# NYXFLOWER/TIP

Measured on AMD Instinct MI355X. Metric: D-D edges aggregated/sec (encoder fwd+bwd), higher is better.
Workload: dtype f32; 1 GPU; TIP-cat full encoder, BioSNAP (645 drugs, 19081 proteins, R=1097), 1xMI355X config; mod=cat, directed_dd_edges=8326508, relations=1097, parallelism=single GPU, launch=hipGraph replay of the captured step, rccl_ranks=0

## Files before the change

### tip_amd/csrc/tipk_gemm.hip

```cpp
#include <stdlib.h>
#include "tipk_common.h"
#include "tipk_slabs.h"

namespace {

typedef float f32x16 __attribute__((ext_vector_type(16)));

constexpr int BK = 32;
constexpr int PAD = 4;

struct GemmArgs {
    int64_t m, n, k, kbatch, ksplit, kchunk;
    const float* a; int64_t a_sm, a_sk, a_sq, a_sz;
    const float* b; int64_t b_sk, b_sn, b_sq, b_sz;
    float* c; int64_t c_sm, c_sz, c_ss;
    const float* c_in; int64_t cin_sm, cin_sz;
    float alpha;
    int relu;
};

typedef unsigned int u32;

__device__ __forceinline__ float ldg(const float* base, u32 byte_off) {
    return *reinterpret_cast<const float*>(reinterpret_cast<const char*>(base) + byte_off);
}
__device__ __forceinline__ float4 ldg4(const float* base, u32 byte_off) {
    return *reinterpret_cast<const float4*>(reinterpret_cast<const char*>(base) + byte_off);
}

template <int ROWS>
struct TileLoader {
    static constexpr int PER = ROWS * BK / 256;
    float v[PER];
    __device__ __forceinline__ static void coord(bool kfast, int i, int t, int& r, int& kk) {
        r = kfast ? t / BK + (256 / BK) * i : t % ROWS;
        kk = kfast ? t % BK : t / ROWS + (256 / ROWS) * i;
    }
    __device__ __forceinline__ void load(bool kfast, const float* tile, u32 s_r, u32 s_k, int rows_left, int k_left, int t) {
#pragma unroll
        for (int i = 0; i < PER; ++i) {
            int r, kk;
            coord(kfast, i, t, r, kk);
            v[i] = (r < rows_left && kk < k_left) ? ldg(tile, ((u32)r * s_r + (u32)kk * s_k) * 4u) : 0.f;
        }
    }
    __device__ __forceinline__ void store(bool kfast, float (*lds)[ROWS + PAD], int t) const {
#pragma unroll
        for (int i = 0; i < PER; ++i) {
            int r, kk;
            coord(kfast, i, t, r, kk);
            lds[kk][r] = v[i];
        }
    }
};

template <int WM, int WN, int NBUF, int R = 1>
__device__ __forceinline__ void gemm_body(const GemmArgs& g, int64_t bx, int64_t by, int64_t bz, float* smem,
                                          const bool A_KFAST, const bool B_KFAST) {
    constexpr int BM = WM * 32 * R, BN = WN * 32 * R;
    static_assert(WM * WN == 4, "4 waves per workgroup");
    float (*As)[BK][BM + PAD] = reinterpret_cast<float (*)[BK][BM + PAD]>(smem);
    float (*Bs)[BK][BN + PAD] = reinterpret_cast<float (*)[BK][BN + PAD]>(smem + NBUF * BK * (BM + PAD));

    const int t = threadIdx.x;
    const int lane = t & 63, wid = t >> 6;
    const int wm = wid / WN, wn = wid % WN;
    const int64_t m0 = by * BM, n0 = bx * BN;
    const int64_t z = bz / g.ksplit, slab = bz % g.ksplit;
    const int64_t k_lo = slab * g.kchunk;
    const int64_t k_hi = (k_lo + g.kchunk < g.k) ? k_lo + g.kchunk : g.k;
    const int tiles_per_q = (k_hi > k_lo) ? (int)((k_hi - k_lo + BK - 1) / BK) : 0;
    const int n_tiles = tiles_per_q * (int)g.kbatch;

    const float* a_z = g.a + z * g.a_sz + m0 * g.a_sm + k_lo * g.a_sk;
    const float* b_z = g.b + z * g.b_sz + n0 * g.b_sn + k_lo * g.b_sk;
    const u32 a_sm = (u32)g.a_sm, a_sk = (u32)g.a_sk, b_sn = (u32)g.b_sn, b_sk = (u32)g.b_sk;
    const int m_left = (int)(g.m - m0 < BM ? g.m - m0 : BM), n_left = (int)(g.n - n0 < BN ? g.n - n0 : BN);

    TileLoader<BM> la;
    TileLoader<BN> lb;
    f32x16 acc[R][R];
#pragma unroll
    for (int a = 0; a < R; ++a)
#pragma unroll
        for (int b = 0; b < R; ++b)
#pragma unroll
            for (int i = 0; i < 16; ++i) acc[a][b][i] = 0.f;

    auto fetch = [&](int tile) {
        const int q = tile / tiles_per_q;
        const int kt = tile - q * tiles_per_q;
        const int k_left = (int)(k_hi - k_lo) - kt * BK;
        la.load(A_KFAST, a_z + (int64_t)q * g.a_sq + (int64_t)kt * BK * g.a_sk, a_sm, a_sk, m_left, k_left, t);
        lb.load(B_KFAST, b_z + (int64_t)q * g.b_sq + (int64_t)kt * BK * g.b_sk, b_sn, b_sk, n_left, k_left, t);
    };

    if (n_tiles > 0) fetch(0);
    for (int tile = 0; tile < n_tiles; ++tile) {
        const int buf = NBUF == 2 ? (tile & 1) : 0;
        if (NBUF == 1 && tile > 0) __syncthreads();
        la.store(A_KFAST, As[buf], t);
        lb.store(B_KFAST, Bs[buf], t);
        __syncthreads();
        if (tile + 1 < n_tiles) fetch(tile + 1);
        const int row = lane & 31, kh = lane >> 5;
#pragma unroll
        for (int kk = 0; kk < BK / 2; ++kk) {
            float av[R], bv[R];
#pragma unroll
            for (int a = 0; a < R; ++a) av[a] = As[buf][2 * kk + kh][(wm * R + a) * 32 + row];
#pragma unroll
            for (int b = 0; b < R; ++b) bv[b] = Bs[buf][2 * kk + kh][(wn * R + b) * 32 + row];
#pragma unroll
            for (int a = 0; a < R; ++a)
#pragma unroll
                for (int b = 0; b < R; ++b)
                    acc[a][b] = __builtin_amdgcn_mfma_f32_32x32x2f32(av[a], bv[b], acc[a][b], 0, 0, 0);
        }
    }

    float* c_z = g.c + z * g.c_sz + slab * g.c_ss;
    const float* cin_z = g.c_in ? g.c_in + z * g.cin_sz : nullptr;
#pragma unroll
    for (int a = 0; a < R; ++a) {
#pragma unroll
        for (int b = 0; b < R; ++b) {
            const int64_t col = n0 + (wn * R + b) * 32 + (lane & 31);
            if (col >= g.n) continue;
#pragma unroll
            for (int r = 0; r < 16; ++r) {
                const int64_t rowi = m0 + (wm * R + a) * 32 + (r & 3) + 8 * (r >> 2) + 4 * (lane >> 5);
                if (rowi < g.m) {
                    float v = g.alpha * acc[a][b][r];
                    if (cin_z) v += cin_z[rowi * g.cin_sm + col];
                    if (g.relu) v = fmaxf(v, 0.f);
                    c_z[rowi * g.c_sm + col] = v;
                }
            }
        }
    }
}

template <int WM, int WN, bool A_KFAST, bool B_KFAST, int NBUF, int R = 1>
__global__ __launch_bounds__(256) void gemm_f32_kernel(GemmArgs g) {
    __shared__ __attribute__((aligned(16))) float smem[NBUF * BK * (WM * 32 * R + WN * 32 * R + 2 * PAD)];
    gemm_body<WM, WN, NBUF, R>(g, blockIdx.x, blockIdx.y, blockIdx.z, smem, A_KFAST, B_KFAST);
}

constexpr int THIN_K_NT = 4;

__device__ __forceinline__ f32x16 zero16() {
    f32x16 z;
#pragma unroll
    for (int i = 0; i < 16; ++i) z[i] = 0.f;
    return z;
}

__device__ __forceinline__ void store_tile(const GemmArgs& g, const f32x16& acc, float* c_z, const float* cin_z,
                                           int64_t m0, int64_t n0, int lane) {
    const int64_t col = n0 + (lane & 31);
    if (col >= g.n) return;
#pragma unroll
    for (int r = 0; r < 16; ++r) {
        const int64_t rowi = m0 + (r & 3) + 8 * (r >> 2) + 4 * (lane >> 5);
        if (rowi < g.m) {
            float v = g.alpha * acc[r];
            if (cin_z) v += cin_z[rowi * g.cin_sm + col];
            if (g.relu) v = fmaxf(v, 0.f);
            c_z[rowi * g.c_sm + col] = v;
        }
    }
}

__device__ __forceinline__ float and_mask(float v, u32 mask) { return __uint_as_float(__float_as_uint(v) & mask); }
__device__ __forceinline__ int uniform(int v) { return __builtin_amdgcn_readfirstlane(v); }

__device__ __forceinline__ void store_tile32(const GemmArgs& g, const f32x16& acc, float* c_z, const float* cin_z,
                                             int m0, int n0, int lane) {
    const int col = n0 + (lane & 31);
    if (col >= (int)g.n) return;
    float* c_t = c_z + (int64_t)m0 * g.c_sm + n0;
    const float* cin_t = cin_z ? cin_z + (int64_t)m0 * g.cin_sm + n0 : nullptr;
    const u32 c_sm = (u32)g.c_sm * 4u, cin_sm = (u32)g.cin_sm * 4u;
    const u32 cb = (u32)(lane & 31) * 4u;
#pragma unroll
    for (int r = 0; r < 16; ++r) {
        const int rl = (r & 3) + 8 * (r >> 2) + 4 * (lane >> 5);
        if (m0 + rl < (int)g.m) {
            float v = g.alpha * acc[r];
            if (cin_t) v += ldg(cin_t, (u32)rl * cin_sm + cb);
            if (g.relu) v = fmaxf(v, 0.f);
            *reinterpret_cast<float*>(reinterpret_cast<char*>(c_t) + ((u32)rl * c_sm + cb)) = v;
        }
    }
}

template <bool WIDE>
__device__ __forceinline__ void gemm_thin_k_body(const GemmArgs& g, int64_t block) {
    const int lane = threadIdx.x & 63;
    const int row = lane & 31, kh = lane >> 5;
    const int M = (int)g.m, N = (int)g.n, K = (int)g.k;
    const int m_tiles = (M + 31) / 32;
    const int n_chunks = (N + 32 * THIN_K_NT - 1) / (32 * THIN_K_NT);
    const int gw = uniform((int)block * 4 + (int)(threadIdx.x >> 6));
    const int z = uniform(gw / (m_tiles * n_chunks));
    const int rem = gw - z * (m_tiles * n_chunks);
    const int chunk = uniform(rem / m_tiles), mt = uniform(rem - chunk * m_tiles);
    if (z >= g.kbatch) return;
    const int m0 = mt * 32;
    const float* __restrict__ a_z = g.a + z * g.a_sz;
    const float* __restrict__ b_z = g.b + z * g.b_sz;
    float* c_z = g.c + z * g.c_sz;
    const float* cin_z = g.c_in ? g.c_in + z * g.cin_sz : nullptr;
    const u32 a_sk = (u32)g.a_sk * 4u, b_sk = (u32)g.b_sk * 4u;
    const u32 aoff = (u32)(m0 + row < M ? m0 + row : M - 1) * (u32)g.a_sm * 4u;
    float av[16];
    u32 koff[16];
    const bool a_vec = WIDE && g.a_sk == 1 && (g.a_sm & 3) == 0 && (g.a_sz & 3) == 0 && K == 32 &&
                       (reinterpret_cast<uintptr_t>(g.a) & 15) == 0;
    if (a_vec) {
#pragma unroll
        for (int q = 0; q < 4; ++q) {
            const float4 t = ldg4(a_z, aoff + (u32)(16 * kh + 4 * q) * 4u);
            av[4 * q + 0] = t.x; av[4 * q + 1] = t.y; av[4 * q + 2] = t.z; av[4 * q + 3] = t.w;
        }
    }
#pragma unroll
    for (int kk = 0; kk < 16; ++kk) {
        const int k = WIDE ? 16 * kh + kk : 2 * kk + kh;
        const u32 kc = (u32)(k < K ? k : K - 1);
        if (!a_vec) av[kk] = and_mask(ldg(a_z, aoff + kc * a_sk), k < K ? 0xffffffffu : 0u);
        koff[kk] = kc * b_sk;
    }
    const int nb = chunk * (32 * THIN_K_NT);
    if (WIDE) {
        const int col = nb + 4 * row;
        const u32 cc = (u32)(col < N ? col : N - 4) * 4u;
        float4 b4[16];
#pragma unroll
        for (int kk = 0; kk < 16; ++kk) b4[kk] = ldg4(b_z, koff[kk] + cc);
        __builtin_amdgcn_sched_barrier(0);
        f32x16 a0 = zero16(), a1 = zero16(), a2 = zero16(), a3 = zero16();
#pragma unroll
        for (int kk = 0; kk < 16; ++kk) {
            a0 = __builtin_amdgcn_mfma_f32_32x32x2f32(av[kk], b4[kk].x, a0, 0, 0, 0);
            a1 = __builtin_amdgcn_mfma_f32_32x32x2f32(av[kk], b4[kk].y, a1, 0, 0, 0);
            a2 = __builtin_amdgcn_mfma_f32_32x32x2f32(av[kk], b4[kk].z, a2, 0, 0, 0);
            a3 = __builtin_amdgcn_mfma_f32_32x32x2f32(av[kk], b4[kk].w, a3, 0, 0, 0);
        }
        if (col >= N) return;
        float* c_t = c_z + (int64_t)m0 * g.c_sm + nb;
        const float* cin_t = cin_z ? cin_z + (int64_t)m0 * g.cin_sm + nb : nullptr;
        const u32 c_sm = (u32)g.c_sm * 4u, cin_sm = (u32)g.cin_sm * 4u, cb = (u32)row * 16u;
#pragma unroll
        for (int r = 0; r < 16; ++r) {
            const int rl = (r & 3) + 8 * (r >> 2) + 4 * kh;
            if (m0 + rl < M) {
                float4 v = make_float4(g.alpha * a0[r], g.alpha * a1[r], g.alpha * a2[r], g.alpha * a3[r]);
                if (cin_t) {
                    const float4 ci = ldg4(cin_t, (u32)rl * cin_sm + cb);
                    v.x += ci.x; v.y += ci.y; v.z += ci.z; v.w += ci.w;
                }
                if (g.relu) { v.x = fmaxf(v.x, 0.f); v.y = fmaxf(v.y, 0.f); v.z = fmaxf(v.z, 0.f); v.w = fmaxf(v.w, 0.f); }
                *reinterpret_cast<float4*>(reinterpret_cast<char*>(c_t) + ((u32)rl * c_sm + cb)) = v;
            }
        }
        return;
    }
    float bt[THIN_K_NT][16];
#pragma unroll
    for (int j = 0; j < THIN_K_NT; ++j) {
        const int col = nb + 32 * j + row;
        const u32 cc = (u32)(col < N ? col : N - 1) * 4u;
#pragma unroll
        for (int kk = 0; kk < 16; ++kk) bt[j][kk] = ldg(b_z, koff[kk] + cc);
    }
    __builtin_amdgcn_sched_barrier(0);
#pragma unroll
    for (int j = 0; j < THIN_K_NT; ++j) {
        f32x16 acc = zero16();
#pragma unroll
        for (int kk = 0; kk < 16; ++kk) acc = __builtin_amdgcn_mfma_f32_32x32x2f32(av[kk], bt[j][kk], acc, 0, 0, 0);
        store_tile32(g, acc, c_z, cin_z, m0, nb + 32 * j, lane);
    }
}

__device__ __forceinline__ void gemm_thin_m_body(const GemmArgs& g, int64_t block) {
    const int lane = threadIdx.x & 63;
    const int row = lane & 31, kh = lane >> 5;
    const int M = (int)g.m, N = (int)g.n;
    const int n_tiles = (N + 31) / 32;
    const int gw = uniform((int)block * 4 + (int)(threadIdx.x >> 6));
    const int zs = uniform(gw / n_tiles);
    const int nt = gw - zs * n_tiles;
    const int z = uniform(zs / (int)g.ksplit);
    const int slab = zs - z * (int)g.ksplit;
    if (z >= g.kbatch) return;
    const int k_lo = slab * (int)g.kchunk;
    const int k_hi = (k_lo + (int)g.kchunk < (int)g.k) ? k_lo + (int)g.kchunk : (int)g.k;
    const float* __restrict__ a_z = g.a + z * g.a_sz;
    const float* __restrict__ b_z = g.b + z * g.b_sz;
    const int n0 = nt * 32;
    const int col = n0 + row;
    const u32 cc = (u32)(col < N ? col : N - 1) * 4u;
    const u32 a_sk = (u32)g.a_sk * 4u, b_sk = (u32)g.b_sk * 4u;
    const u32 ar = (u32)(row < M ? row : M - 1) * (u32)g.a_sm * 4u;
    float a0[16], b0[16], a1[16], b1[16];
#define TIPK_LOAD_AB(A, B, K0)                                                 \
    _Pragma("unroll") for (int kk = 0; kk < 16; ++kk) {                        \
        const int k_ = (K0) + 2 * kk + kh;                                     \
        const u32 kc_ = (u32)(k_ < k_hi ? k_ : k_hi - 1);                      \
        A[kk] = ldg(a_z, ar + kc_ * a_sk);                                     \
        B[kk] = ldg(b_z, kc_ * b_sk + cc);                                     \
    }                                                                          \
    __builtin_amdgcn_sched_barrier(0);
#define TIPK_MMA(A, B, K0)                                                     \
    _Pragma("unroll") for (int kk = 0; kk < 16; ++kk)                          \
        acc = __builtin_amdgcn_mfma_f32_32x32x2f32(and_mask(A[kk], (K0) + 2 * kk + kh < k_hi ? 0xffffffffu : 0u), \
                                                   B[kk], acc, 0, 0, 0);       \
    __builtin_amdgcn_sched_barrier(0);
    f32x16 acc = zero16();
    if (k_lo < k_hi) {
        TIPK_LOAD_AB(a0, b0, k_lo)
#pragma unroll 1
        for (int k0 = k_lo; k0 < k_hi; k0 += 64) {
            TIPK_LOAD_AB(a1, b1, k0 + 32)
            TIPK_MMA(a0, b0, k0)
            TIPK_LOAD_AB(a0, b0, k0 + 64)
            TIPK_MMA(a1, b1, k0 + 32)
        }
    }
#undef TIPK_LOAD_AB
#undef TIPK_MMA
    float* c_z = g.c + z * g.c_sz + (int64_t)slab * g.c_ss;
    const float* cin_z = g.c_in ? g.c_in + z * g.cin_sz : nullptr;
    store_tile32(g, acc, c_z, cin_z, 0, n0, lane);
}

__device__ __forceinline__ void gemm_kk_body(const GemmArgs& g, int64_t block) {
    const int lane = threadIdx.x & 63;
    const int row = lane & 31, kh = lane >> 5;
    const int M = (int)g.m, N = (int)g.n;
    const int m_tiles = (M + 31) / 32;
    const int gw = uniform((int)block * 4 + (int)(threadIdx.x >> 6));
    const int zs = uniform(gw / m_tiles);
    const int mt = gw - zs * m_tiles;
    const int z = uniform(zs / (int)g.ksplit);
    const int slab = zs - z * (int)g.ksplit;
    if (z >= g.kbatch) return;
    const int k_lo = slab * (int)g.kchunk;
    const int k_hi = (k_lo + (int)g.kchunk < (int)g.k) ? k_lo + (int)g.kchunk : (int)g.k;
    const int m0 = mt * 32;
    const float* __restrict__ a_z = g.a + z * g.a_sz;
    const float* __restrict__ b_z = g.b + z * g.b_sz;
    const u32 ar = (u32)(m0 + row < M ? m0 + row : M - 1) * (u32)g.a_sm * 4u;
    const u32 br = (u32)(row < N ? row : N - 1) * (u32)g.b_sn * 4u;
    float4 a0[4], b0[4], a1[4], b1[4];
#define TIPK_LOAD_AB(A, B, K0)                                                 \
    _Pragma("unroll") for (int q = 0; q < 4; ++q) {                            \
        const int k_ = (K0) + 8 * q + 4 * kh;                                  \
        const u32 kc_ = (u32)(k_ < k_hi ? k_ : k_hi - 4) * 4u;                 \
        A[q] = ldg4(a_z, ar + kc_);                                            \
        B[q] = ldg4(b_z, br + kc_);                                            \
    }                                                                          \
    __builtin_amdgcn_sched_barrier(0);
#define TIPK_KK_STEP(A, B, K0)                                                 \
    _Pragma("unroll") for (int q = 0; q < 4; ++q) {                            \
        const u32 mk_ = (K0) + 8 * q + 4 * kh < k_hi ? 0xffffffffu : 0u;       \
        acc = __builtin_amdgcn_mfma_f32_32x32x2f32(and_mask(A[q].x, mk_), B[q].x, acc, 0, 0, 0); \
        acc = __builtin_amdgcn_mfma_f32_32x32x2f32(and_mask(A[q].y, mk_), B[q].y, acc, 0, 0, 0); \
        acc = __builtin_amdgcn_mfma_f32_32x32x2f32(and_mask(A[q].z, mk_), B[q].z, acc, 0, 0, 0); \
        acc = __builtin_amdgcn_mfma_f32_32x32x2f32(and_mask(A[q].w, mk_), B[q].w, acc, 0, 0, 0); \
    }                                                                          \
    __builtin_amdgcn_sched_barrier(0);
    f32x16 acc = zero16();
    if (k_lo < k_hi) {
        TIPK_LOAD_AB(a0, b0, k_lo)
#pragma unroll 1
        for (int k0 = k_lo; k0 < k_hi; k0 += 64) {
            TIPK_LOAD_AB(a1, b1, k0 + 32)
            TIPK_KK_STEP(a0, b0, k0)
            TIPK_LOAD_AB(a0, b0, k0 + 64)
            TIPK_KK_STEP(a1, b1, k0 + 32)
        }
    }
#undef TIPK_LOAD_AB
#undef TIPK_KK_STEP
    float* c_z = g.c + z * g.c_sz + (int64_t)slab * g.c_ss;
    const float* cin_z = g.c_in ? g.c_in + z * g.cin_sz : nullptr;
    store_tile32(g, acc, c_z, cin_z, m0, 0, lane);
}

enum { STREAM_NONE = 0, STREAM_THIN_K = 1, STREAM_THIN_M = 2, STREAM_KK = 3, STREAM_THIN_K4 = 4 };

inline bool thin_k_wide_ok(const GemmArgs& g, int64_t batch) {
    static_assert(THIN_K_NT == 4, "the wide body owns four interleaved tiles");
    if ((g.n & 3) || ((g.b_sk | g.c_sm | g.b_sz | g.c_sz) & 3)) return false;
    if (g.c_in && ((g.cin_sm | g.cin_sz) & 3)) return false;
    return ((reinterpret_cast<uintptr_t>(g.b) | reinterpret_cast<uintptr_t>(g.c) | reinterpret_cast<uintptr_t>(g.c_in)) & 15) == 0;
}

inline int stream_kind(const GemmArgs& g, int64_t batch) {
    if (g.kbatch != 1) return STREAM_NONE;
    const bool big = g.m * g.n >= (1 << 20) || g.n * g.k >= (1 << 20) || g.m * g.k >= (1 << 20);
    if (!big) return STREAM_NONE;
    const int64_t lim = 0x3fffffffLL;
    if (g.a_sm < 0 || g.a_sk < 0 || g.b_sk < 0 || g.b_sn < 0 || g.m > lim || g.n > lim || g.k > lim) return STREAM_NONE;
    if ((g.m - 1) * g.a_sm + (g.k - 1) * g.a_sk >= lim || (g.k - 1) * g.b_sk + (g.n - 1) * g.b_sn >= lim) return STREAM_NONE;
    if (g.c_sm < 0 || g.cin_sm < 0 || 32 * g.c_sm >= lim || 32 * g.cin_sm >= lim) return STREAM_NONE;
    if (g.k <= 32 && g.ksplit == 1 && g.b_sn == 1 && (g.m >= 256 || (g.m >= 8 && g.n >= (1 << 16))) && g.n >= 1024)
        return (thin_k_wide_ok(g, batch) && !tipk_option(TIPK_OPT_GEMM_THIN_K_NARROW)) ? STREAM_THIN_K4 : STREAM_THIN_K;
    if (g.m <= 32 && g.b_sn == 1 && g.n >= 1024 && g.k >= 256) return STREAM_THIN_M;
    if (tipk_option(TIPK_OPT_GEMM_STREAM_KK) && g.n <= 32 && g.a_sk == 1 && g.b_sk == 1 && g.m >= 256 && g.k >= 1024 && g.k % 4 == 0 && g.a_sm % 4 == 0 &&
        g.b_sn % 4 == 0 && g.a_sz % 4 == 0 && g.b_sz % 4 == 0 && (reinterpret_cast<uintptr_t>(g.a) & 15) == 0 &&
        (reinterpret_cast<uintptr_t>(g.b) & 15) == 0)
        return STREAM_KK;
    return STREAM_NONE;
}

inline int64_t stream_blocks(int kind, const GemmArgs& g, int64_t batch) {
    int64_t waves = 0;
    if (kind == STREAM_THIN_K || kind == STREAM_THIN_K4) waves = batch * tipk_ceil_div(g.m, 32) * tipk_ceil_div(g.n, 32 * THIN_K_NT);
    if (kind == STREAM_THIN_M) waves = batch * g.ksplit * tipk_ceil_div(g.n, 32);
    if (kind == STREAM_KK) waves = batch * g.ksplit * tipk_ceil_div(g.m, 32);
    return tipk_ceil_div(waves, 4);
}

template <int KIND>
__global__ __launch_bounds__(256) void gemm_stream_kernel(GemmArgs g) {
    if (KIND == STREAM_THIN_K) gemm_thin_k_body<false>(g, blockIdx.x);
    if (KIND == STREAM_THIN_K4) gemm_thin_k_body<true>(g, blockIdx.x);
    if (KIND == STREAM_THIN_M) gemm_thin_m_body(g, blockIdx.x);
    if (KIND == STREAM_KK) gemm_kk_body(g, blockIdx.x);
}

constexpr int GROUP_MAX = TIPK_GROUP_MAX;

struct GemmGroupArgs {
    int count;
    int first_block[GROUP_MAX + 1];
    int cfg[GROUP_MAX];
    int gx[GROUP_MAX], gy[GROUP_MAX];
    GemmArgs g[GROUP_MAX];
};

__global__ __launch_bounds__(256) void gemm_f32_group_kernel(GemmGroupArgs ga) {
    __shared__ __attribute__((aligned(16))) float smem[2 * BK * (160 + 2 * PAD)];
    GemmArgs g = ga.g[0];
    int first = 0, gx = ga.gx[0], gy = ga.gy[0], cfg = ga.cfg[0];
#pragma unroll
    for (int q = 1; q < GROUP_MAX; ++q)
        if (q < ga.count && (int)blockIdx.x >= ga.first_block[q]) {
            g = ga.g[q]; first = ga.first_block[q]; gx = ga.gx[q]; gy = ga.gy[q]; cfg = ga.cfg[q];
        }
    const int local = (int)blockIdx.x - first;
    const int64_t bx = local % gx, by = (local / gx) % gy, bz = local / (gx * gy);
    const bool akf = (cfg & 2) != 0, bkf = (cfg & 1) != 0;
    switch (cfg >= 100 ? cfg : cfg >> 2) {
    case 0: gemm_body<4, 1, 2>(g, bx, by, bz, smem, akf, bkf); break;
    case 1: gemm_body<1, 4, 2>(g, bx, by, bz, smem, akf, bkf); break;
    case 2: gemm_body<2, 2, 2>(g, bx, by, bz, smem, akf, bkf); break;
    case 100 + STREAM_THIN_M: gemm_thin_m_body(g, local); break;
    case 100 + STREAM_KK: gemm_kk_body(g, local); break;
    }
}

template <int WM, int WN, int R = 1>
int launch(const GemmArgs& g, int64_t batch, hipStream_t st) {
    constexpr int BM = WM * 32 * R, BN = WN * 32 * R;
    const int64_t gx = tipk_ceil_div(g.n, BN), gy = tipk_ceil_div(g.m, BM), gz = batch * g.ksplit;
    if (gx > 0x7fffffffLL || gy > 65535 || gz > 65535) return TIPK_EUNSUPPORTED;
    dim3 grid((unsigned)gx, (unsigned)gy, (unsigned)gz), block(256);
    const bool akf = g.a_sk == 1 || g.a_sm != 1;
    const bool bkf = g.b_sk == 1 && g.b_sn != 1;
    const bool one_tile = g.kbatch == 1 && g.kchunk <= BK;
#define TIPK_GEMM_GO(A, B)                                                                              \
    do {                                                                                                \
        if (one_tile) hipLaunchKernelGGL((gemm_f32_kernel<WM, WN, A, B, 1, R>), grid, block, 0, st, g); \
        else hipLaunchKernelGGL((gemm_f32_kernel<WM, WN, A, B, (R > 1 ? 1 : 2), R>), grid, block, 0, st, g); \
    } while (0)
    if (akf && bkf) TIPK_GEMM_GO(true, true);
    else if (akf) TIPK_GEMM_GO(true, false);
    else if (bkf) TIPK_GEMM_GO(false, true);
    else TIPK_GEMM_GO(false, false);
#undef TIPK_GEMM_GO
    TIPK_RETURN_LAUNCH();
}

template <int LANES>
__global__ __launch_bounds__(64 * LANES) void sum_slabs_kernel(const float* __restrict__ in, int64_t n_slabs,
                                                               int64_t slab_stride, int64_t count, float alpha,
                                                               int accumulate, const float* __restrict__ row_scale,
                                                               int64_t cols, const float* __restrict__ addend,
                                                               int relu, float* __restrict__ out) {
    __shared__ float red[LANES][64];
    const int e = threadIdx.x & 63, j = threadIdx.x >> 6;
    const int64_t i = (int64_t)blockIdx.x * 64 + e;
    float s = 0.f;
    if (i < count) {
        const float* p = in + i;
        int64_t k = j;
        for (; k + 3 * LANES < n_slabs; k += 4 * LANES) {
            const float v0 = p[k * slab_stride], v1 = p[(k + LANES) * slab_stride];
            const float v2 = p[(k + 2 * LANES) * slab_stride], v3 = p[(k + 3 * LANES) * slab_stride];
            s += v0; s += v1; s += v2; s += v3;
        }
        for (; k < n_slabs; k += LANES) s += p[k * slab_stride];
    }
    red[j][e] = s;
    __syncthreads();
    if (j == 0 && i < count) {
        s = red[0][e];
#pragma unroll
        for (int q = 1; q < LANES; ++q) s += red[q][e];
        s *= alpha;
        if (row_scale) s *= row_scale[i / cols];
        if (addend) s += addend[i];
        if (accumulate) s += out[i];
        if (relu) s = fmaxf(s, 0.f);
        out[i] = s;
    }
}

struct SlabGroupArgs {
    int count;
    int first_block[GROUP_MAX + 1];
    SlabArgs s[GROUP_MAX];
};

__global__ __launch_bounds__(1024) void sum_slabs_group_kernel(SlabGroupArgs sa) {
    __shared__ float red[1024];
    SlabArgs a = sa.s[0];
    int first = 0;
#pragma unroll
    for (int q = 1; q < GROUP_MAX; ++q)
        if (q < sa.count && (int)blockIdx.x >= sa.first_block[q]) { a = sa.s[q]; first = sa.first_block[q]; }
    slab_sum_body(a, (int)blockIdx.x - first, red);
}

constexpr int WGK_MAX = 4, WGK_SUMS = 3, WGK_WAVES = 16;

struct WgkJob {
    const float* a; int64_t a_sm, a_sk, a_sq, a_sz;
    const float* b; int64_t b_sk, b_sn, b_sq, b_sz;
    const float* a2; int64_t a2_sm, a2_sk;
    const float* b2; int64_t b2_sk, b2_sn;
    float* c; int64_t c_sm, c_sz;
    const float* c_in; int64_t cin_sm, cin_sz;
    const float* gate; int64_t gate_sm, gate_sz;
    int m, n, k, k2, kbatch;
    int mt, nt;
    int tiles_q, n_kt, per, nw;
    int vec1, vec2;
    float alpha; int relu;
};
struct WgkArgs {
    int n_gemm, n_sum;
    int first[WGK_MAX + WGK_SUMS + 1];
    WgkJob g[WGK_MAX];
    SlabArgs s[WGK_SUMS];
};

__global__ __launch_bounds__(1024) void gemm_wgk_group_kernel(WgkArgs wa) {
    __shared__ __attribute__((aligned(16))) float red[WGK_WAVES * 1024];
    const int blk = (int)blockIdx.x;
    if (blk >= wa.first[WGK_MAX]) {
        SlabArgs sa = wa.s[0];
        int first = wa.first[WGK_MAX];
#pragma unroll
        for (int q = 1; q < WGK_SUMS; ++q)
            if (q < wa.n_sum && blk >= wa.first[WGK_MAX + q]) { sa = wa.s[q]; first = wa.first[WGK_MAX + q]; }
        slab_sum_body(sa, blk - first, red);
        return;
    }
    WgkJob g = wa.g[0];
    int first = 0;
#pragma unroll
    for (int q = 1; q < WGK_MAX; ++q)
        if (q < wa.n_gemm && blk >= wa.first[q]) { g = wa.g[q]; first = wa.first[q]; }
    const int local = blk - first;
    const int nt_i = local % g.nt, mt_i = (local / g.nt) % g.mt, z = local / (g.nt * g.mt);
    const int t = threadIdx.x, lane = t & 63, row = lane & 31, kh = lane >> 5;
    const int w = uniform(t >> 6);
    const int m0 = mt_i * 32, n0 = nt_i * 32;
    const int n_first = g.kbatch * g.tiles_q;
    const u32 am = (u32)(m0 + row < g.m ? m0 + row : g.m - 1), bn = (u32)(n0 + row < g.n ? n0 + row : g.n - 1);
    const u32 m_mask = m0 + row < g.m ? 0xffffffffu : 0u;

    f32x16 acc = zero16();
    float a0[16], b0[16], a1[16], b1[16];
    int left0 = 0, left1 = 0;
    auto load = [&](int tile, float (&av)[16], float (&bv)[16], int& left) {
        const bool second = tile >= n_first;
        const int tq = second ? tile - n_first : tile;
        const int q = second ? 0 : tq / g.tiles_q;
        const int kt = second ? tq : tq - q * g.tiles_q;
        const int kk_total = second ? g.k2 : g.k;
        const int k0 = kt * 32;
        left = kk_total - k0 < 32 ? kk_total - k0 : 32;
        const float* ap = second ? g.a2 : g.a + (int64_t)z * g.a_sz + (int64_t)q * g.a_sq;
        const float* bp = second ? g.b2 : g.b + (int64_t)z * g.b_sz + (int64_t)q * g.b_sq;
        const u32 s_am = (u32)(second ? g.a2_sm : g.a_sm), s_ak = (u32)(second ? g.a2_sk : g.a_sk);
        const u32 s_bk = (u32)(second ? g.b2_sk : g.b_sk), s_bn = (u32)(second ? g.b2_sn : g.b_sn);
        const u32 ao = am * s_am, bo = bn * s_bn;
        if (second ? g.vec2 : g.vec1) {
#pragma unroll
            for (int j = 0; j < 4; ++j) {
                const int kb = 16 * kh + 4 * j;
                const u32 kc = (u32)(k0 + (kb < left ? kb : left - 4));
                const float4 xa = ldg4(ap, (ao + kc) * 4u), xb = ldg4(bp, (bo + kc) * 4u);
                av[4 * j] = xa.x; av[4 * j + 1] = xa.y; av[4 * j + 2] = xa.z; av[4 * j + 3] = xa.w;
                bv[4 * j] = xb.x; bv[4 * j + 1] = xb.y; bv[4 * j + 2] = xb.z; bv[4 * j + 3] = xb.w;
            }
            left = -left;
            return;
        }
#pragma unroll
        for (int kk = 0; kk < 16; ++kk) {
            const int kl = 2 * kk + kh;
            const u32 kc = (u32)(k0 + (kl < left ? kl : left - 1));
            av[kk] = ldg(ap, (ao + kc * s_ak) * 4u);
            bv[kk] = ldg(bp, (kc * s_bk + bo) * 4u);
        }
    };
    auto mma = [&](const float (&av)[16], const float (&bv)[16], int left) {
        const int lim = left < 0 ? -left - 16 * kh : left - kh;
        const int step = left < 0 ? 1 : 2;
#pragma unroll
        for (int kk = 0; kk < 16; ++kk)
            acc = __builtin_amdgcn_mfma_f32_32x32x2f32(and_mask(av[kk], step * kk < lim ? m_mask : 0u), bv[kk], acc, 0, 0, 0);
    };
    const int t_lo = w * g.per, t_hi = t_lo + g.per < g.n_kt ? t_lo + g.per : g.n_kt;
    if (t_lo < t_hi) {
        load(t_lo, a0, b0, left0);
#pragma unroll 1
        for (int tile = t_lo; tile < t_hi; tile += 2) {
            if (tile + 1 < t_hi) load(tile + 1, a1, b1, left1);
            __builtin_amdgcn_sched_barrier(0);
            mma(a0, b0, left0);
            __builtin_amdgcn_sched_barrier(0);
            if (tile + 1 < t_hi) {
                if (tile + 2 < t_hi) load(tile + 2, a0, b0, left0);
                __builtin_amdgcn_sched_barrier(0);
                mma(a1, b1, left1);
                __builtin_amdgcn_sched_barrier(0);
            }
        }
#pragma unroll
        for (int r = 0; r < 16; ++r) red[w * 1024 + r * 64 + lane] = acc[r];
    }
    __syncthreads();
    {
        float s = g.nw > 0 ? red[t] : 0.f;
        for (int q = 1; q < g.nw; ++q) s += red[q * 1024 + t];
        const int r = t >> 6, l = t & 63;
        const int rr = m0 + (r & 3) + 8 * (r >> 2) + 4 * (l >> 5), cc = n0 + (l & 31);
        if (rr < g.m && cc < g.n) {
            s *= g.alpha;
            if (g.c_in) s += g.c_in[(int64_t)z * g.cin_sz + (int64_t)rr * g.cin_sm + cc];
            if (g.relu) s = fmaxf(s, 0.f);
            if (g.gate && !(g.gate[(int64_t)z * g.gate_sz + (int64_t)rr * g.gate_sm + cc] > 0.f)) s = 0.f;
            g.c[(int64_t)z * g.c_sz + (int64_t)rr * g.c_sm + cc] = s;
        }
    }
}

}

static int fill_args(const tipk_gemm_desc* d, GemmArgs& g) {
    if (!d || d->m < 0 || d->n < 0 || d->k < 0 || d->batch < 0 || d->kbatch < 1 || d->ksplit < 1) return TIPK_EINVAL;
    if (d->m == 0 || d->n == 0 || d->batch == 0) return 1;
    if (!d->a || !d->b || !d->c) return TIPK_EINVAL;
    if (d->ksplit > 1 && (d->c_in || d->relu)) return TIPK_EINVAL;
    if (d->a_sm < 0 || d->a_sk < 0 || d->b_sk < 0 || d->b_sn < 0) return TIPK_EINVAL;
    if (128 * d->a_sm + 32 * d->a_sk >= (1LL << 30) || 128 * d->b_sn + 32 * d->b_sk >= (1LL << 30)) return TIPK_EUNSUPPORTED;
    g.m = d->m; g.n = d->n; g.k = d->k; g.kbatch = d->kbatch; g.ksplit = d->ksplit;
    g.kchunk = tipk_ceil_div(tipk_ceil_div(d->k, d->ksplit), BK) * BK;
    if (g.kchunk == 0) g.kchunk = BK;
    g.a = d->a; g.a_sm = d->a_sm; g.a_sk = d->a_sk; g.a_sq = d->a_sq; g.a_sz = d->a_sz;
    g.b = d->b; g.b_sk = d->b_sk; g.b_sn = d->b_sn; g.b_sq = d->b_sq; g.b_sz = d->b_sz;
    g.c = d->c; g.c_sm = d->c_sm; g.c_sz = d->c_sz; g.c_ss = d->c_ss;
    g.c_in = d->c_in; g.cin_sm = d->cin_sm; g.cin_sz = d->cin_sz;
    g.alpha = d->alpha; g.relu = d->relu;
    return TIPK_OK;
}

extern "C" int tipk_gemm_f32(const tipk_gemm_desc* d, tipk_stream_t stream) {
    GemmArgs g;
    const int rc = fill_args(d, g);
    if (rc != TIPK_OK) return rc > 0 ? TIPK_OK : rc;
    hipStream_t st = (hipStream_t)stream;
    const int kind = tipk_option(TIPK_OPT_GEMM_NO_STREAM) ? STREAM_NONE : stream_kind(g, d->batch);
    if (kind != STREAM_NONE) {
        const int64_t blocks = stream_blocks(kind, g, d->batch);
        if (blocks > 0x7fffffffLL) return TIPK_EUNSUPPORTED;
        g.kbatch = d->batch;
        if (kind == STREAM_THIN_K)
            hipLaunchKernelGGL(gemm_stream_kernel<STREAM_THIN_K>, dim3((unsigned)blocks), dim3(256), 0, st, g);
        else if (kind == STREAM_THIN_K4)
            hipLaunchKernelGGL(gemm_stream_kernel<STREAM_THIN_K4>, dim3((unsigned)blocks), dim3(256), 0, st, g);
        else if (kind == STREAM_THIN_M)
            hipLaunchKernelGGL(gemm_stream_kernel<STREAM_THIN_M>, dim3((unsigned)blocks), dim3(256), 0, st, g);
        else
            hipLaunchKernelGGL(gemm_stream_kernel<STREAM_KK>, dim3((unsigned)blocks), dim3(256), 0, st, g);
        TIPK_RETURN_LAUNCH();
    }
    if (d->n <= 32) return launch<4, 1>(g, d->batch, st);
    if (d->m <= 32) return launch<1, 4>(g, d->batch, st);
    if (d->m >= 512 && d->n >= 512 && d->ksplit == 1) return launch<2, 2, 2>(g, d->batch, st);
    return launch<2, 2>(g, d->batch, st);
}

extern "C" int tipk_gemm_f32_group(const tipk_gemm_desc* descs, int32_t count, tipk_stream_t stream) {
    if (count < 0 || count > GROUP_MAX || (count > 0 && !descs)) return TIPK_EINVAL;
    GemmGroupArgs ga;
    ga.count = 0;
    int64_t blocks = 0;
    const bool no_stream = tipk_option(TIPK_OPT_GEMM_NO_STREAM) != 0;
    for (int i = 0; i < count; ++i) {
        GemmArgs& g = ga.g[ga.count];
        const int rc = fill_args(descs + i, g);
        if (rc < 0) return rc;
        if (rc > 0) continue;
        int kind = no_stream ? STREAM_NONE : stream_kind(g, descs[i].batch);
        if (kind == STREAM_THIN_K || kind == STREAM_THIN_K4) kind = STREAM_NONE;
        if (kind != STREAM_NONE) {
            const int64_t nb = stream_blocks(kind, g, descs[i].batch);
            if (nb > 0x3fffffffLL) return TIPK_EUNSUPPORTED;
            g.kbatch = descs[i].batch;
            ga.cfg[ga.count] = 100 + kind;
            ga.gx[ga.count] = 1;
            ga.gy[ga.count] = 1;
            ga.first_block[ga.count] = (int)blocks;
            blocks += nb;
            if (blocks > 0x3fffffffLL) return TIPK_EUNSUPPORTED;
            ++ga.count;
            continue;
        }
        const int shape = g.n <= 32 ? 0 : (g.m <= 32 ? 1 : 2);
        const int bm = shape == 0 ? 128 : (shape == 1 ? 32 : 64), bn = shape == 0 ? 32 : (shape == 1 ? 128 : 64);
        const bool akf = g.a_sk == 1 || g.a_sm != 1;
        const bool bkf = g.b_sk == 1 && g.b_sn != 1;
        const int64_t gx = tipk_ceil_div(g.n, bn), gy = tipk_ceil_div(g.m, bm), gz = descs[i].batch * g.ksplit;
        if (gx > 0x7fffffLL || gy > 65535 || gz > 65535 || gx * gy * gz > 0x3fffffffLL) return TIPK_EUNSUPPORTED;
        ga.cfg[ga.count] = shape * 4 + (akf ? 2 : 0) + (bkf ? 1 : 0);
        ga.gx[ga.count] = (int)gx;
        ga.gy[ga.count] = (int)gy;
        ga.first_block[ga.count] = (int)blocks;
        blocks += gx * gy * gz;
        if (blocks > 0x3fffffffLL) return TIPK_EUNSUPPORTED;
        ++ga.count;
    }
    if (ga.count == 0) return TIPK_OK;
    ga.first_block[ga.count] = (int)blocks;
    hipLaunchKernelGGL(gemm_f32_group_kernel, dim3((unsigned)blocks), dim3(256), 0, (hipStream_t)stream, ga);
    TIPK_RETURN_LAUNCH();
}

extern "C" int tipk_sum_slabs_group(const tipk_slab_sum_desc* descs, int32_t count, tipk_stream_t stream) {
    if (count < 0 || count > GROUP_MAX || (count > 0 && !descs)) return TIPK_EINVAL;
    SlabGroupArgs sa;
    sa.count = 0;
    int64_t blocks = 0;
    for (int i = 0; i < count; ++i) {
        int rc;
        const int64_t nb = fill_slab_args(descs[i], sa.s[sa.count], &rc);
        if (rc != TIPK_OK) return rc;
        if (nb == 0) continue;
        sa.first_block[sa.count] = (int)blocks;
        blocks += nb;
        if (blocks > 0x3fffffffLL) return TIPK_EUNSUPPORTED;
        ++sa.count;
    }
    if (sa.count == 0) return TIPK_OK;
    sa.first_block[sa.count] = (int)blocks;
    hipLaunchKernelGGL(sum_slabs_group_kernel, dim3((unsigned)blocks), dim3(1024), 0, (hipStream_t)stream, sa);
    TIPK_RETURN_LAUNCH();
}

static int fill_wgk(const tipk_wg_gemm_desc& d, WgkJob& j) {
    const tipk_gemm_desc& p = d.p;
    if (p.m <= 0 || p.n <= 0 || p.k < 0 || p.batch <= 0 || p.kbatch < 1 || p.ksplit != 1) return TIPK_EINVAL;
    if (!p.a || !p.b || !p.c || p.a_sm < 0 || p.a_sk < 0 || p.b_sk < 0 || p.b_sn < 0) return TIPK_EINVAL;
    const bool second = d.a2 != nullptr;
    if (second && (!d.b2 || d.k2 <= 0 || p.batch != 1 || d.a2_sm < 0 || d.a2_sk < 0 || d.b2_sk < 0 || d.b2_sn < 0)) return TIPK_EINVAL;
    const int64_t lim = 1LL << 30;
    if (p.m > lim || p.n > lim || p.k > lim || p.m * p.a_sm + p.k * p.a_sk >= lim || p.k * p.b_sk + p.n * p.b_sn >= lim) return TIPK_EUNSUPPORTED;
    if (second && (d.k2 > lim || p.m * d.a2_sm + d.k2 * d.a2_sk >= lim || d.k2 * d.b2_sk + p.n * d.b2_sn >= lim)) return TIPK_EUNSUPPORTED;
    const int64_t tiles_q = tipk_ceil_div(p.k, 32);
    const int64_t n_kt = p.kbatch * tiles_q + (second ? tipk_ceil_div(d.k2, 32) : 0);
    const int64_t mt = tipk_ceil_div(p.m, 32), nt = tipk_ceil_div(p.n, 32);
    if (n_kt < 1 || n_kt > WGK_WAVES * 4 || mt * nt * p.batch > 4096) return TIPK_EUNSUPPORTED;
    j.a = p.a; j.a_sm = p.a_sm; j.a_sk = p.a_sk; j.a_sq = p.a_sq; j.a_sz = p.a_sz;
    j.b = p.b; j.b_sk = p.b_sk; j.b_sn = p.b_sn; j.b_sq = p.b_sq; j.b_sz = p.b_sz;
    j.a2 = d.a2; j.a2_sm = d.a2_sm; j.a2_sk = d.a2_sk; j.b2 = d.b2; j.b2_sk = d.b2_sk; j.b2_sn = d.b2_sn;
    j.c = p.c; j.c_sm = p.c_sm; j.c_sz = p.c_sz;
    j.c_in = p.c_in; j.cin_sm = p.cin_sm; j.cin_sz = p.cin_sz;
    j.gate = d.gate; j.gate_sm = d.gate_sm; j.gate_sz = d.gate_sz;
    j.m = (int)p.m; j.n = (int)p.n; j.k = (int)p.k; j.k2 = second ? (int)d.k2 : 0; j.kbatch = (int)p.kbatch;
    j.mt = (int)mt; j.nt = (int)nt;
    j.tiles_q = (int)tiles_q; j.n_kt = (int)n_kt;
    j.per = (int)tipk_ceil_div(n_kt, WGK_WAVES);
    j.nw = (int)tipk_ceil_div(n_kt, j.per);
    j.alpha = p.alpha; j.relu = p.relu;
    const auto al16 = [](const void* q) { return (reinterpret_cast<uintptr_t>(q) & 15) == 0; };
    j.vec1 = p.a_sk == 1 && p.b_sk == 1 && p.k % 4 == 0 && ((p.a_sm | p.b_sn | p.a_sq | p.b_sq | p.a_sz | p.b_sz) & 3) == 0 && al16(p.a) && al16(p.b);
    j.vec2 = second && d.a2_sk == 1 && d.b2_sk == 1 && d.k2 % 4 == 0 && ((d.a2_sm | d.b2_sn) & 3) == 0 && al16(d.a2) && al16(d.b2);
    return TIPK_OK;
}

extern "C" int tipk_gemm_wg_group_supported(const tipk_wg_gemm_desc* d) {
    WgkJob j;
    return d && fill_wgk(*d, j) == TIPK_OK;
}

extern "C" int tipk_gemm_wg_group(const tipk_wg_gemm_desc* descs, int32_t count, const tipk_slab_sum_desc* sums,
                                  int32_t n_sums, tipk_stream_t stream) {
    if (count < 0 || count > WGK_MAX || n_sums < 0 || n_sums > WGK_SUMS || (count > 0 && !descs) || (n_sums > 0 && !sums)) return TIPK_EINVAL;
    WgkArgs wa;
    wa.n_gemm = count; wa.n_sum = 0;
    int64_t blocks = 0;
    for (int i = 0; i < count; ++i) {
        const int rc = fill_wgk(descs[i], wa.g[i]);
        if (rc != TIPK_OK) return rc;
        wa.first[i] = (int)blocks;
        blocks += (int64_t)wa.g[i].mt * wa.g[i].nt * descs[i].p.batch;
    }
    for (int i = count; i <= WGK_MAX; ++i) wa.first[i] = (int)blocks;
    for (int i = 0; i < n_sums; ++i) {
        int rc;
        const int64_t nb = fill_slab_args(sums[i], wa.s[wa.n_sum], &rc);
        if (rc != TIPK_OK) return rc;
        if (nb == 0) continue;
        wa.first[WGK_MAX + wa.n_sum] = (int)blocks;
        blocks += nb;
        if (blocks > 0x3fffffffLL) return TIPK_EUNSUPPORTED;
        ++wa.n_sum;
    }
    for (int i = wa.n_sum; i <= WGK_SUMS; ++i) wa.first[WGK_MAX + i] = (int)blocks;
    if (blocks == 0) return TIPK_OK;
    hipLaunchKernelGGL(gemm_wgk_group_kernel, dim3((unsigned)blocks), dim3(1024), 0, (hipStream_t)stream, wa);
    TIPK_RETURN_LAUNCH();
}

extern "C" int tipk_sum_slabs_ex(const float* in, int64_t n_slabs, int64_t slab_stride, int64_t count, float alpha,
                                 int accumulate, const float* row_scale, int64_t cols, const float* addend, int relu,
                                 float* out, tipk_stream_t stream) {
    if (n_slabs < 0 || count < 0 || (row_scale && cols <= 0)) return TIPK_EINVAL;
    if (count == 0) return TIPK_OK;
    if (!out || (n_slabs > 0 && !in)) return TIPK_EINVAL;
    const int64_t blocks = tipk_ceil_div(count, 64);
    if (blocks > 0x7fffffffLL) return TIPK_EUNSUPPORTED;
    if (n_slabs >= 32 && blocks < 2048)
        hipLaunchKernelGGL(sum_slabs_kernel<16>, dim3((unsigned)blocks), dim3(1024), 0, (hipStream_t)stream, in, n_slabs,
                           slab_stride, count, alpha, accumulate, row_scale, cols, addend, relu, out);
    else
        hipLaunchKernelGGL(sum_slabs_kernel<4>, dim3((unsigned)blocks), dim3(256), 0, (hipStream_t)stream, in, n_slabs,
                           slab_stride, count, alpha, accumulate, row_scale, cols, addend, relu, out);
    TIPK_RETURN_LAUNCH();
}

extern "C" int tipk_sum_slabs(const float* in, int64_t n_slabs, int64_t slab_stride, int64_t count, float alpha,
                              int accumulate, float* out, tipk_stream_t stream) {
    return tipk_sum_slabs_ex(in, n_slabs, slab_stride, count, alpha, accumulate, nullptr, 0, nullptr, 0, out, stream);
}
```

Measured before the change: 39.75 billion edges/s.

## Balance split-K tiles across waves, unroll the load pipeline, prefetch epilogue operands

The grouped split-K GEMM kernel now spreads K tiles across its 16 waves with a per/rem split, so wave loads differ by at most one tile. The ping-pong loop is replaced by a fully unrolled sequence of up to four tiles, issuing three tile loads before the first MFMA. The c_in and gate values for the epilogue are loaded before the barrier so their latency overlaps the main loop, and the cross-wave reduction is unrolled by four. Row masking of A is dropped because rows are clamped and stores are masked. Debug switches for skipping loads, MFMAs, reductions and stores are also added, which costs extra registers and runtime branches on a uniform flag.

```diff
diff --git a/tip_amd/csrc/tipk_gemm.hip b/tip_amd/csrc/tipk_gemm.hip
--- a/tip_amd/csrc/tipk_gemm.hip
+++ b/tip_amd/csrc/tipk_gemm.hip
@@ -550,12 +550,14 @@
     const float* gate; int64_t gate_sm, gate_sz;
     int m, n, k, k2, kbatch;
     int mt, nt;
-    int tiles_q, n_kt, per, nw;
+    int tiles_q, n_kt;
+    int per, rem, nw;
     int vec1, vec2;
     float alpha; int relu;
 };
 struct WgkArgs {
     int n_gemm, n_sum;
+    int dbg;
     int first[WGK_MAX + WGK_SUMS + 1];
     WgkJob g[WGK_MAX];
     SlabArgs s[WGK_SUMS];
@@ -585,11 +587,19 @@
     const int m0 = mt_i * 32, n0 = nt_i * 32;
     const int n_first = g.kbatch * g.tiles_q;
     const u32 am = (u32)(m0 + row < g.m ? m0 + row : g.m - 1), bn = (u32)(n0 + row < g.n ? n0 + row : g.n - 1);
-    const u32 m_mask = m0 + row < g.m ? 0xffffffffu : 0u;
+
+    const int er = m0 + (w & 3) + 8 * (w >> 2) + 4 * kh, ec = n0 + row;
+    const bool e_ok = er < g.m && ec < g.n;
+    const int64_t erc = er < g.m ? er : g.m - 1, ecc = ec < g.n ? ec : g.n - 1;
+    float e_cin = 0.f, e_gate = 1.f;
+    if (!TIPK_DBG(wa.dbg & 8)) {
+        if (g.c_in) e_cin = g.c_in[(int64_t)z * g.cin_sz + erc * g.cin_sm + ecc];
+        if (g.gate) e_gate = g.gate[(int64_t)z * g.gate_sz + erc * g.gate_sm + ecc];
+    }
 
     f32x16 acc = zero16();
-    float a0[16], b0[16], a1[16], b1[16];
-    int left0 = 0, left1 = 0;
+    float a0[16], b0[16], a1[16], b1[16], a2[16], b2[16];
+    int left0 = 0, left1 = 0, left2 = 0;
     auto load = [&](int tile, float (&av)[16], float (&bv)[16], int& left) {
         const bool second = tile >= n_first;
         const int tq = second ? tile - n_first : tile;
@@ -598,12 +608,20 @@
         const int kk_total = second ? g.k2 : g.k;
         const int k0 = kt * 32;
         left = kk_total - k0 < 32 ? kk_total - k0 : 32;
+        const bool vec = second ? g.vec2 : g.vec1;
+        if (TIPK_DBG(wa.dbg & 1)) {
+#pragma unroll
+            for (int kk = 0; kk < 16; ++kk) { av[kk] = 0.f; bv[kk] = 0.f; }
+            if (vec) left = -left;
+            return;
+        }
         const float* ap = second ? g.a2 : g.a + (int64_t)z * g.a_sz + (int64_t)q * g.a_sq;
         const float* bp = second ? g.b2 : g.b + (int64_t)z * g.b_sz + (int64_t)q * g.b_sq;
-        const u32 s_am = (u32)(second ? g.a2_sm : g.a_sm), s_ak = (u32)(second ? g.a2_sk : g.a_sk);
-        const u32 s_bk = (u32)(second ? g.b2_sk : g.b_sk), s_bn = (u32)(second ? g.b2_sn : g.b_sn);
+        const u32 m2 = second ? 0xffffffffu : 0u, m1 = ~m2;
+        const u32 s_am = ((u32)g.a2_sm & m2) | ((u32)g.a_sm & m1), s_ak = ((u32)g.a2_sk & m2) | ((u32)g.a_sk & m1);
+        const u32 s_bk = ((u32)g.b2_sk & m2) | ((u32)g.b_sk & m1), s_bn = ((u32)g.b2_sn & m2) | ((u32)g.b_sn & m1);
         const u32 ao = am * s_am, bo = bn * s_bn;
-        if (second ? g.vec2 : g.vec1) {
+        if (vec) {
 #pragma unroll
             for (int j = 0; j < 4; ++j) {
                 const int kb = 16 * kh + 4 * j;
@@ -624,43 +642,61 @@
         }
     };
     auto mma = [&](const float (&av)[16], const float (&bv)[16], int left) {
+        if (TIPK_DBG(wa.dbg & 2)) {
+            acc[0] += av[0] + bv[0] + av[15] + bv[15];
+            return;
+        }
         const int lim = left < 0 ? -left - 16 * kh : left - kh;
         const int step = left < 0 ? 1 : 2;
 #pragma unroll
         for (int kk = 0; kk < 16; ++kk)
-            acc = __builtin_amdgcn_mfma_f32_32x32x2f32(and_mask(av[kk], step * kk < lim ? m_mask : 0u), bv[kk], acc, 0, 0, 0);
+            acc = __builtin_amdgcn_mfma_f32_32x32x2f32(and_mask(av[kk], step * kk < lim ? 0xffffffffu : 0u), bv[kk], acc, 0, 0, 0);
     };
-    const int t_lo = w * g.per, t_hi = t_lo + g.per < g.n_kt ? t_lo + g.per : g.n_kt;
-    if (t_lo < t_hi) {
+    const int t_lo = w * g.per + (w < g.rem ? w : g.rem), cnt = g.per + (w < g.rem ? 1 : 0);
+    if (cnt > 0) {
         load(t_lo, a0, b0, left0);
-#pragma unroll 1
-        for (int tile = t_lo; tile < t_hi; tile += 2) {
-            if (tile + 1 < t_hi) load(tile + 1, a1, b1, left1);
-            __builtin_amdgcn_sched_barrier(0);
-            mma(a0, b0, left0);
-            __builtin_amdgcn_sched_barrier(0);
-            if (tile + 1 < t_hi) {
-                if (tile + 2 < t_hi) load(tile + 2, a0, b0, left0);
-                __builtin_amdgcn_sched_barrier(0);
-                mma(a1, b1, left1);
-                __builtin_amdgcn_sched_barrier(0);
+        if (cnt > 1) load(t_lo + 1, a1, b1, left1);
+        if (cnt > 2) load(t_lo + 2, a2, b2, left2);
+        __builtin_amdgcn_sched_barrier(0);
+        mma(a0, b0, left0);
+        __builtin_amdgcn_sched_barrier(0);
+        if (cnt > 3) load(t_lo + 3, a0, b0, left0);
+        __builtin_amdgcn_sched_barrier(0);
+        if (cnt > 1) mma(a1, b1, left1);
+        if (cnt > 2) mma(a2, b2, left2);
+        __builtin_amdgcn_sched_barrier(0);
+        if (cnt > 3) mma(a0, b0, left0);
+        if (!TIPK_DBG(wa.dbg & 4)) {
+#pragma unroll
+            for (int r = 0; r < 16; ++r) red[w * 1024 + r * 64 + lane] = acc[r];
+        }
+    }
+    __syncthreads();
+    asm volatile("" : "+v"(e_gate));
+    {
+        float s;
+        if (TIPK_DBG(wa.dbg & 4)) {
+            s = acc[0];
+        } else {
+            s = 0.f;
+#pragma unroll
+            for (int q = 0; q < WGK_WAVES; q += 4) {
+                if (q < g.nw) {
+                    const float v0 = red[q * 1024 + t], v1 = red[(q + 1) * 1024 + t];
+                    const float v2 = red[(q + 2) * 1024 + t], v3 = red[(q + 3) * 1024 + t];
+                    s = q == 0 ? v0 : s + v0;
+                    if (q + 1 < g.nw) s += v1;
+                    if (q + 2 < g.nw) s += v2;
+                    if (q + 3 < g.nw) s += v3;
+                }
             }
         }
-#pragma unroll
-        for (int r = 0; r < 16; ++r) red[w * 1024 + r * 64 + lane] = acc[r];
-    }
-    __syncthreads();
-    {
-        float s = g.nw > 0 ? red[t] : 0.f;
-        for (int q = 1; q < g.nw; ++q) s += red[q * 1024 + t];
-        const int r = t >> 6, l = t & 63;
-        const int rr = m0 + (r & 3) + 8 * (r >> 2) + 4 * (l >> 5), cc = n0 + (l & 31);
-        if (rr < g.m && cc < g.n) {
+        if (e_ok) {
             s *= g.alpha;
-            if (g.c_in) s += g.c_in[(int64_t)z * g.cin_sz + (int64_t)rr * g.cin_sm + cc];
+            if (g.c_in) s += e_cin;
             if (g.relu) s = fmaxf(s, 0.f);
-            if (g.gate && !(g.gate[(int64_t)z * g.gate_sz + (int64_t)rr * g.gate_sm + cc] > 0.f)) s = 0.f;
-            g.c[(int64_t)z * g.c_sz + (int64_t)rr * g.c_sm + cc] = s;
+            if (g.gate && !(e_gate > 0.f)) s = 0.f;
+            if (!TIPK_DBG(wa.dbg & 16)) g.c[(int64_t)z * g.c_sz + (int64_t)er * g.c_sm + ec] = s;
         }
     }
 }
@@ -800,8 +836,8 @@
     j.m = (int)p.m; j.n = (int)p.n; j.k = (int)p.k; j.k2 = second ? (int)d.k2 : 0; j.kbatch = (int)p.kbatch;
     j.mt = (int)mt; j.nt = (int)nt;
     j.tiles_q = (int)tiles_q; j.n_kt = (int)n_kt;
-    j.per = (int)tipk_ceil_div(n_kt, WGK_WAVES);
-    j.nw = (int)tipk_ceil_div(n_kt, j.per);
+    j.per = (int)(n_kt / WGK_WAVES); j.rem = (int)(n_kt % WGK_WAVES);
+    j.nw = (int)(n_kt < WGK_WAVES ? n_kt : WGK_WAVES);
     j.alpha = p.alpha; j.relu = p.relu;
     const auto al16 = [](const void* q) { return (reinterpret_cast<uintptr_t>(q) & 15) == 0; };
     j.vec1 = p.a_sk == 1 && p.b_sk == 1 && p.k % 4 == 0 && ((p.a_sm | p.b_sn | p.a_sq | p.b_sq | p.a_sz | p.b_sz) & 3) == 0 && al16(p.a) && al16(p.b);
@@ -819,6 +855,7 @@
     if (count < 0 || count > WGK_MAX || n_sums < 0 || n_sums > WGK_SUMS || (count > 0 && !descs) || (n_sums > 0 && !sums)) return TIPK_EINVAL;
     WgkArgs wa;
     wa.n_gemm = count; wa.n_sum = 0;
+    wa.dbg = TIPK_DBG(tipk_option(TIPK_OPT_DP_DEBUG));
     int64_t blocks = 0;
     for (int i = 0; i < count; ++i) {
         const int rc = fill_wgk(descs[i], wa.g[i]);
```

New measurement: 40.22 billion edges/s (median of 6 runs). 1.2% higher.
